# RegulatoryGenomicsGroup/chicdiff

Hardware: AMD Instinct MI355X
Metric: interactions/sec NB-GLM Wald test (higher is better)
Workload: dtype f64; 1 GPU; synthetic 2000000 interactions x 8 samples (4v4), size factors + offsets(theta=0.5) + dispersions + Wald, design ~condition; rows_per_gpu=2000000, samples=8, global_rows=2000000, parallelism=rows-sharded x1, collectives=none (single rank), ranks_in_communicator=1

## Files before the change

chicdiff_amd/csrc/api.hip:

```cpp
#include <math.h>
#include <stdarg.h>
#include <stdio.h>
#include <stdlib.h>
#include <string.h>

#include <algorithm>
#include <mutex>
#include <thread>
#include <string>
#include <vector>
#include <unordered_set>

#include <dlfcn.h>

#include "common.h"
#include "philox.h"
#include "prior_mc.h"

using namespace cd;

namespace cd {
struct ChinputCols {
    std::vector<int32_t> bait, oe, N;
    std::string error;
};
int64_t chinput_parse(const char *path, int nthreads, ChinputCols &c);
}

struct KTimer {
    std::string name;
    hipEvent_t e0 = nullptr, e1 = nullptr;
    double ms = 0;
    int launches = 0;
    double bytes = 0;
};

struct HostOpts {
    int select_all_rounds = 0;
    int trend_one_launch_per_pass = 0;
    int sharded_trend_gather = 1;
    int trend_mad_in_kernel = 1;
    int local_trend_substitute = 1;
    int fuse_offsets = 1;
    int prep_blocks = 0;
    int theta_grid_concurrency = 5;
    int host_copy_threads = 12;
    int bench_fake_world = 0;
    int fault_inject = 0;
    int region_assemble_generic = 0;
    int chicago_tables_run_merge = 1;
};

struct chicdiff_hip_ctx {
    int device = 0;
    bool no_persistent_trend = false;
    Opts tune{};
    HostOpts host;
    char *tg_buf = nullptr;
    size_t tg_bytes = 0;
    double shard_n[kSelMaxWorld] = {0};
    bool shard_n_valid = false;
    int64_t tg_total = 0;
    double *tg_x = nullptr, *tg_y = nullptr, *tg_resid = nullptr;
    int32_t *tg_flags = nullptr;
    int32_t *h_flag = nullptr;
    FusedOffsets fuse;
    int refits = 0;
    bool sf_overflow_seen = false;
    int32_t *d_carry = nullptr;
    char *io_dev = nullptr, *io_pin = nullptr;
    size_t io_dev_bytes = 0, io_pin_bytes = 0;
    ChinputCols *chin = nullptr;
    struct EarlyCopy {
        int n = 0;
        struct Item { int col; char *pin; size_t bytes; } item[10];
        hipEvent_t ready = nullptr, done = nullptr;
        bool issued = false;
    } *early = nullptr;
    hipStream_t copy_stream = nullptr;
    hipEvent_t ev_fork = nullptr, ev_join = nullptr;
    std::vector<chicdiff_hip_ctx *> lanes;
    int cu_count = 0;
    hipStream_t own_stream = nullptr, stream = nullptr;
    chicdiff_allreduce_fn allreduce = nullptr;
    void *allreduce_user = nullptr;
    chicdiff_allgather_fn allgather = nullptr;
    void *allgather_user = nullptr;
    int world = 1, rank = 0;
    void *rccl_lib = nullptr, *rccl_comm = nullptr;
    int (*rccl_allreduce)(const void *, void *, size_t, int, int, void *, hipStream_t) = nullptr;
    int (*rccl_allgather)(const void *, void *, size_t, int, void *, hipStream_t) = nullptr;
    int (*rccl_comm_destroy)(void *) = nullptr;
    const char *(*rccl_error_string)(int) = nullptr;
    char err[512] = {0};
    int64_t cap_n = 0;
    int cap_S = 0;
    void *ws = nullptr;
// ... 39 lines not shown
    va_end(ap);
    return code;
}
#define HIPCHK(c, call)                                                                              \
    do {                                                                                             \
        hipError_t e_ = (call);                                                                      \
        if (e_ != hipSuccess) return fail(c, CHICDIFF_E_HIP, "%s: %s", #call, hipGetErrorString(e_)); \
    } while (0)

extern "C" {

const char *chicdiff_hip_last_error(const chicdiff_hip_ctx *ctx) { return ctx ? ctx->err : g_create_err; }

void chicdiff_hip_default_opts(chicdiff_nbglm_opts *o) {
    o->minDisp = 1e-8;
    o->dispTol = 1e-6;
    o->kappa0 = 1.0;
    o->maxit = 100;
    o->betaMaxit = 100;
    o->betaTol = 1e-8;
    o->minmu = 0.5;
    o->outlierSD = 2.0;
    o->dispPriorVar = NAN;
    o->trendCoef[0] = o->trendCoef[1] = NAN;
    o->fitType = 0;
    o->_pad = 0;
}

struct OptionDef {
    const char *name;
    int32_t Opts::*tune;
    int HostOpts::*host;
    int64_t lo, hi, no_lo, no_hi;
};
static const OptionDef kOptions[] = {
    {"line_search_spread", &Opts::spread, nullptr, 0, 3, 1, 0},
    {"line_search_min_waves", &Opts::min_waves, nullptr, 0, 4, 1, 1},
    {"line_search_chunk", &Opts::chunk, nullptr, 0, 64, 1, 7},
    {"line_search_prio", &Opts::prio, nullptr, 0, 100, 1, 0},
    {"line_search_schedule", &Opts::schedule, nullptr, 0, 4, 2, 2},
    {"line_search_deal", &Opts::deal, nullptr, 0, 64, 1, 0},
    {"line_search_classes_a", &Opts::classes_a, nullptr, 0, 6, 1, 0},
    {"line_search_fillers", &Opts::fillers, nullptr, -1, 1, 1, 0},
    {"line_search_filler_stop", &Opts::filler_stop, nullptr, -1, 100, 1, 0},
    {"theta_grid_concurrency", nullptr, &HostOpts::theta_grid_concurrency, 1, 16, 1, 0},
    {"host_copy_threads", nullptr, &HostOpts::host_copy_threads, 1, 64, 1, 0},
    {"select_all_rounds", nullptr, &HostOpts::select_all_rounds, 0, 1, 1, 0},
    {"trend_one_launch_per_pass", nullptr, &HostOpts::trend_one_launch_per_pass, 0, 1, 1, 0},
    {"sharded_trend_gather", nullptr, &HostOpts::sharded_trend_gather, 0, 1, 1, 0},
    {"trend_persistent_blocks", &Opts::trend_blocks, nullptr, 0, 256, 1, 0},
    {"trend_mad_in_kernel", nullptr, &HostOpts::trend_mad_in_kernel, 0, 1, 1, 0},
    {"fuse_offsets", nullptr, &HostOpts::fuse_offsets, 0, 2, 1, 0},
    {"prep_blocks", nullptr, &HostOpts::prep_blocks, 0, kRedBlocks, 1, 0},
    {"region_assemble_generic", nullptr, &HostOpts::region_assemble_generic, 0, 1, 1, 0},
    {"chicago_tables_run_merge", nullptr, &HostOpts::chicago_tables_run_merge, 0, 1, 1, 0},
    {"fault_inject", nullptr, &HostOpts::fault_inject, 0, 7, 1, 0},
    {"bench_fake_world", nullptr, &HostOpts::bench_fake_world, 0, kGatherMaxWorld, 1, 0},
    {"local_trend_substitute", nullptr, &HostOpts::local_trend_substitute, 0, 1, 1, 0},
};

int chicdiff_hip_set_option(chicdiff_hip_ctx *c, const char *name, int64_t value) {
    if (!c || !name) return CHICDIFF_E_INVALID;
    for (const OptionDef &d : kOptions) {
        if (strcmp(name, d.name) != 0 || value < d.lo || value > d.hi || (value >= d.no_lo && value <= d.no_hi)) continue;
        if (d.host == &HostOpts::bench_fake_world && value > 1 && !getenv("CHICDIFF_BENCH_FAKE_WORLD"))
            return fail(c, CHICDIFF_E_INVALID, "set_option: bench_fake_world is a rehearsal hook of bench.py (CHICDIFF_BENCH_FAKE_WORLD unset)");
        if (d.tune) c->tune.*d.tune = (int32_t)value;
        else c->host.*d.host = (int)value;
        return CHICDIFF_OK;
    }
    return fail(c, CHICDIFF_E_INVALID, "set_option: unknown option or value (%s = %lld)", name, (long long)value);
}

int chicdiff_hip_create(chicdiff_hip_ctx **out, int32_t device) {
    if (!out) return fail(nullptr, CHICDIFF_E_INVALID, "ctx out pointer is NULL");
    *out = nullptr;
    int ndev = 0;
    hipError_t e = hipGetDeviceCount(&ndev);
    if (e != hipSuccess || ndev <= 0)
        return fail(nullptr, CHICDIFF_E_HIP, "no HIP device available (%s): the HIP path cannot run, and there is no CPU fallback",
                    e != hipSuccess ? hipGetErrorString(e) : "device count 0");
    if (device < 0 || device >= ndev) return fail(nullptr, CHICDIFF_E_INVALID, "device %d out of range [0,%d)", device, ndev);
    chicdiff_hip_ctx *c = new chicdiff_hip_ctx();
    c->device = device;
    if ((e = hipSetDevice(device)) != hipSuccess || (e = hipStreamCreateWithFlags(&c->own_stream, hipStreamNonBlocking)) != hipSuccess ||
        (e = hipHostMalloc((void **)&c->h_sc, sizeof(FitScalars))) != hipSuccess ||
        (e = hipHostMalloc((void **)&c->h_sf, sizeof(double) * (kMaxS + 1))) != hipSuccess ||
        (e = hipMalloc((void **)&c->d_sf, sizeof(double) * (kMaxS + 1 + kSelMaxWorld + 8))) != hipSuccess ||
        (e = hipMemset(c->d_sf, 0, sizeof(double) * (kMaxS + 1 + kSelMaxWorld + 8))) != hipSuccess ||
        (e = hipMalloc((void **)&c->d_logfact, sizeof(double) * kLogFactN)) != hipSuccess) {
        fail(nullptr, CHICDIFF_E_HIP, "context setup: %s", hipGetErrorString(e));
        delete c;
        return CHICDIFF_E_HIP;
    }
    {
        hipDeviceProp_t prop;
        if (hipGetDeviceProperties(&prop, device) == hipSuccess) c->cu_count = prop.multiProcessorCount;
    }
    {
        std::vector<double> lf(kLogFactN);
        for (int k = 0; k < kLogFactN; k++) lf[k] = lgamma((double)k + 1.0);
        if ((e = hipMemcpy(c->d_logfact, lf.data(), sizeof(double) * kLogFactN, hipMemcpyHostToDevice)) != hipSuccess) {
            fail(nullptr, CHICDIFF_E_HIP, "context setup: %s", hipGetErrorString(e));
            chicdiff_hip_destroy(c);
            return CHICDIFF_E_HIP;
        }
// ... 786 lines not shown
    }
    if (c->host.fault_inject & 2) {
        c->host.fault_inject &= ~2;
        launch_poke(&w.sc->failed, 3, st);
    }
    const bool mad_local = c->allreduce && c->tg_total > 0;
    FitDims dm = d;
    FitWork wm = w;
    if (mad_local) {
        dm.n = c->tg_total;
        wm.baseMean = c->tg_x;
        wm.dispGene = c->tg_y;
        wm.allZero = c->tg_flags;
        wm.resid = c->tg_resid;
    }
    if (mad_in_kernel) {
        if (prior_by_simulation(d, o) && (rc = prior_mc(c, d, dm, wm, mad_local))) return rc;
    } else {
        launch_dispfit_resid(dm, wm, o, st);
        SelArgs sa{};
        sa.n = dm.n;
        sa.ncol = 1;
        sa.resid = wm.resid;
        Scope t(c, "mad_select");
        sa.mode = SEL_RESID;
        if ((rc = run_select(c, sa, all_rounds, mad_local))) return rc;
        sa.mode = SEL_ABSDEV;
        if ((rc = run_select(c, sa, all_rounds, mad_local))) return rc;
        if (!prior_by_simulation(d, o)) launch_prior_var(d, w, o, st);
        else if ((rc = prior_mc(c, d, dm, wm, mad_local))) return rc;
    }
    if (c->host.fault_inject & 1) {
        c->host.fault_inject &= ~1;
        launch_poke(&w.sc->sel_overflow, 1, st);
    }
    {
        Scope t(c, "disp_map");
        launch_disp_map(d_counts, d_nf, d, w, o, st);
    }
    if (c->early && c->early->n > 0) {
        const void *src[10] = {w.baseMean, w.baseVar, w.dispGene, w.dispFit, w.dispMAP, w.disp, w.geneIter, w.mapIter, w.outlier, w.allZero};
        HIPCHK(c, hipEventRecord(c->early->ready, st));
        HIPCHK(c, hipStreamWaitEvent(c->copy_stream, c->early->ready, 0));
        for (int k = 0; k < c->early->n; k++)
            HIPCHK(c, hipMemcpyAsync(c->early->item[k].pin, src[c->early->item[k].col], c->early->item[k].bytes, hipMemcpyDeviceToHost, c->copy_stream));
        HIPCHK(c, hipEventRecord(c->early->done, c->copy_stream));
        c->early->issued = true;
    }
    static const chicdiff_nbglm_out none{};
    const chicdiff_nbglm_out &out = d_out ? *d_out : none;
    if (d.p == 2) {
        {
            Scope t(c, "wald_prep");
            launch_wald_prep(d_counts, d_nf, d, w, o, st);
        }
        {
            Scope t(c, "wald_irls");
            launch_wald_irls(d_counts, d_nf, d, w, o, st);
        }
        Scope t(c, "wald_final");
        launch_wald_final(d_counts, d_nf, d, w, o, out, st);
    } else {
        Scope t(c, "wald_intercept");
        launch_wald_intercept(d_counts, d_nf, d, w, o, out, st);
    }
    launch_dev_sum_finish(d, w, c->d_carry, c->d_sf, st);
    if ((rc = do_allreduce(c, w.sc->final_sums, 7))) return rc;
    if ((rc = read_scalars(c))) return rc;
    HIPCHK(c, hipGetLastError());
    return CHICDIFF_OK;
}

static int fit_dev_impl(chicdiff_hip_ctx *c, const int32_t *d_counts, const double *d_nf, FitDims d, Opts o,
                        const chicdiff_nbglm_out *d_out, chicdiff_nbglm_scalars *scalars, bool all_rounds) {
    WorkRedirect redirect(c, d_out);
    const double *hs = c->h_sc->final_sums;
    for (;;) {
        if (int rc = fit_pass(c, d_counts, d_nf, d, o, d_out, all_rounds)) return rc;
        if (hs[4] > 0)
            return fail(c, CHICDIFF_E_INVALID, c->h_sc->neg_counts ? "counts contain a negative value or NA_integer_"
                                                                   : "counts contain a negative value or NA_integer_ (on another rank of the sharded fit)");
        c->sf_overflow_seen = hs[6] > 0;
        if (c->sf_overflow_seen && !all_rounds) return CHICDIFF_OK;
        if (hs[5] > 0 && !all_rounds) {
            all_rounds = true;
        } else if (c->h_sc->failed == 3 || hs[3] > 0) {
            if (c->no_persistent_trend) return fail(c, CHICDIFF_E_HIP, "trend fit: grid barrier timed out");
            c->no_persistent_trend = true;
        } else if (c->h_sc->failed && o.fit_type == 0 && !(o.trendIn[0] == o.trendIn[0]) && c->host.local_trend_substitute) {
            o.fit_type = 2;
        } else
            break;
        c->refits++;
    }
    if (scalars) {
        const FitScalars *s = c->h_sc;
        int status = 0;
        if (s->failed) status |= CHICDIFF_ST_TREND_FAILED;
        if (s->trend_local) status |= CHICDIFF_ST_TREND_LOCAL;
        scalars->trendCoef[0] = s->coefs[0];
        scalars->trendCoef[1] = s->coefs[1];
        scalars->varLogDispEsts = s->varLogDispEsts;
        scalars->dispPriorVar = s->dispPriorVar;
        scalars->nAllZero = (int64_t)hs[2];
        scalars->sumDeviance = hs[2] > 0 ? NAN : hs[0];
        scalars->trendOuterIter = s->outer_it;
        if (hs[2] > 0) status |= CHICDIFF_ST_ALLZERO_ROWS;
        if (hs[1] > 0) status |= CHICDIFF_ST_BETA_NONCONV;
        if (prior_by_simulation(d, o)) status |= CHICDIFF_ST_PRIORVAR_MC;
        scalars->status = status;
    }
    return CHICDIFF_OK;
}

static int begin_call(chicdiff_hip_ctx *c, int rc, int64_t n, int32_t S) {
    timing_reset(c);
    if ((rc = shard_consensus(c, rc, n))) return rc;
// ... 1091 lines not shown
```

chicdiff_amd/csrc/common.h:

```cpp
#pragma once
#include <hip/hip_runtime.h>
#include <stdint.h>

#include "../../include/chicdiff_hip.h"
#include "fit_driver.h"
#include "fit_state.h"

namespace cd {

constexpr int kRedBlocks = 1024;

struct FitDims {
    int64_t n;
    int32_t S, p, nA, nB;
    uint64_t gmask;
};

struct FitWork {
    double *baseMean, *baseVar, *gm0, *gm1, *rough, *binit0, *binit1, *crow;
    double *dispGene, *dispFit, *dispMAP, *disp, *beta0, *beta1, *resid;
    int32_t *allZero, *geneIter, *mapIter, *outlier, *betaIter, *optimConv;
    int32_t *order;
    uint8_t *cls;
    int32_t *gridlist;
// ... 94 lines not shown
    __shared__ unsigned int s_cnt[NC];
    if (threadIdx.x < NC) s_cnt[threadIdx.x] = 0;
    __syncthreads();
#pragma unroll
    for (int k = 0; k < NC; k++) {
        unsigned int v = mine[k];
        for (int off = 32; off > 0; off >>= 1) v += __shfl_down(v, off);
        if ((threadIdx.x & 63) == 0 && v) atomicAdd(&s_cnt[k], v);
    }
    __syncthreads();
    if (threadIdx.x < NC) hist[threadIdx.x * kSchedBlocks + blockIdx.x] = s_cnt[threadIdx.x];
}
__device__ __forceinline__ void class_peers(int c, bool valid, int lane, unsigned int &rank, unsigned int &count) {
    unsigned long long m = __ballot(valid);
#pragma unroll
    for (int b = 0; b < 5; b++) {
        const bool bit = (c >> b) & 1;
        const unsigned long long set = __ballot(bit);
        m &= bit ? set : ~set;
    }
    rank = __popcll(m & ((1ull << lane) - 1ull));
    count = __popcll(m);
}
#endif

struct FusedOffsets { const double *fm = nullptr; const double *sf = nullptr; double theta = 0; int mix = 0; };
int launch_prep(const int32_t *counts, double *nf, FitDims d, FitWork w, Opts o, hipStream_t st, FusedOffsets fo = FusedOffsets(), int max_blocks = 0);
void launch_prep_finish(FitDims d, FitWork w, int nblk, double *slot, hipStream_t st);
void launch_xim(FitDims d, FitWork w, const double *slots, int world, hipStream_t st);
void launch_disp_gene(const int32_t *counts, const double *nf, FitDims d, FitWork w, Opts o, hipStream_t st);
void launch_order_build(FitDims d, FitWork w, int classesA, bool have_hist, hipStream_t st, bool fine = false);
void launch_disp_map(const int32_t *counts, const double *nf, FitDims d, FitWork w, Opts o, hipStream_t st);
void launch_trend_persistent(FitDims d, FitWork w, Opts o, hipStream_t st, bool with_mad);
int trend_persistent_blocks();
void launch_trend_init(FitDims d, FitWork w, Opts o, hipStream_t st);
int trend_blocks();
void launch_trend_pass(FitDims d, FitWork w, Opts o, hipStream_t st, bool fused_step);
void launch_trend_step(FitDims d, FitWork w, Opts o, hipStream_t st);
constexpr int kLfMaxV = 100;
struct LfVerts { int nv; int _pad; double x[kLfMaxV], f[kLfMaxV], d[kLfMaxV]; };
void launch_lf_hist(FitDims d, FitWork w, Opts o, int use_dist, double xv, uint64_t prefix, int shift, double *hist, hipStream_t st);
void launch_lf_sums(FitDims d, FitWork w, Opts o, double xv, double h, double *partials, double *out8, hipStream_t st);
void launch_lf_eval(FitDims d, FitWork w, const LfVerts &v, hipStream_t st);
void launch_trend_gather(FitDims d, FitWork w, Opts o, double *xg, double *yg, hipStream_t st);
constexpr int kGatherMaxWorld = 64;
struct GatherLayout { int32_t world, _pad; int64_t block, maxn; int64_t off[kGatherMaxWorld + 1]; };
void launch_trend_compact(const GatherLayout &gl, const double *recv, double *xg, double *yg, hipStream_t st);
void launch_poke(int32_t *p, int32_t v, hipStream_t st);
void launch_flag_to_double(const int32_t *flag, double *out, hipStream_t st);
void launch_dispfit_resid(FitDims d, FitWork w, Opts o, hipStream_t st);
void launch_prior_var(FitDims d, FitWork w, Opts o, hipStream_t st);
void launch_resid_hist(FitDims d, FitWork w, double *out40, hipStream_t st);
void launch_prior_mc(FitDims d, FitWork w, const double *hist40, const void *table, hipStream_t st);
void launch_wald_prep(const int32_t *counts, const double *nf, FitDims d, FitWork w, Opts o, hipStream_t st);
void launch_wald_irls(const int32_t *counts, const double *nf, FitDims d, FitWork w, Opts o, hipStream_t st);
void launch_wald_final(const int32_t *counts, const double *nf, FitDims d, FitWork w, Opts o,
                       const chicdiff_nbglm_out &out, hipStream_t st);
void launch_wald_intercept(const int32_t *counts, const double *nf, FitDims d, FitWork w, Opts o,
                           const chicdiff_nbglm_out &out, hipStream_t st);
void launch_dev_sum_finish(FitDims d, FitWork w, const int32_t *carry, const double *sf_dev, hipStream_t st);

struct SelArgs {
    int mode;
    int ncol;
    int64_t n;
    const double *resid;
    const double *ratio;
    int S;
    int shift;
    double *sf_out;
    int32_t *overflow_out;
};
void launch_sel_hist(SelArgs a, FitWork w, hipStream_t st);
void launch_sel_step(SelArgs a, FitWork w, hipStream_t st);
void launch_sel_shortcut(SelArgs a, FitWork w, hipStream_t st);
void launch_sel_finish(SelArgs a, FitWork w, hipStream_t st);
void launch_sel_keep_local(SelArgs a, FitWork w, hipStream_t st);
void launch_sel_gather_counts(SelArgs a, FitWork w, int world, int rank, hipStream_t st);
void launch_sel_gather_place(SelArgs a, FitWork w, int world, int rank, hipStream_t st);
void launch_sel_gather_finish(SelArgs a, FitWork w, int world, int rank, hipStream_t st);

void launch_row_ratio(const int32_t *counts, int64_t n, int S, double *ratio, int32_t *clear_flag, hipStream_t st);

constexpr double kSfBinLo = -4.0, kSfBinSpan = 8.0;
constexpr int kSfHistWords = 15360;
constexpr int kSfSubBins = 4096;
constexpr int kSfMaxS = 16;
constexpr int kSfWorkWords = kSfHistWords + 2 * kSfMaxS * 32;
__host__ __device__ inline int sf_bins(int S) { return kSfHistWords / (S <= 4 ? 4 : S <= 8 ? 8 : 16); }
__host__ __device__ inline double sf_bin_pos(double x, int nb) { return (x - kSfBinLo) * ((double)nb / kSfBinSpan); }
__host__ __device__ inline int sf_bin(double x, int nb) {
    const double u = floor(sf_bin_pos(x, nb));
    return u < 0.0 ? 0 : (u > (double)(nb - 1) ? nb - 1 : (int)u);
}
__host__ __device__ inline int sf_sub_bin(double x, int nb, int b) {
    const double u = floor((sf_bin_pos(x, nb) - (double)b) * (double)kSfSubBins);
    return u < 0.0 ? 0 : (u > (double)(kSfSubBins - 1) ? kSfSubBins - 1 : (int)u);
}
void launch_sf_direct(const int32_t *counts, int64_t n, int S, SelArgs a, FitWork w, unsigned int *hist, uint64_t *lists,
                      int32_t *clear_flag, int cus, hipStream_t st);
void launch_offsets(const double *fullMean, const double *sf_dev, int64_t n, int S, double theta, int mix,
                    double *out, hipStream_t st);
void launch_window_sums(const int32_t *fragN, const double *fragFM, int64_t nfrag, int S, const int64_t *rptr,
                        int64_t n, int32_t *N, double *FM, hipStream_t st);
size_t count_join_scratch_bytes(int64_t nkeys);
void launch_count_join(const int32_t *bait, const int32_t *oe, int64_t nru, const int64_t *keys,
                       const int32_t *vals, int64_t nkeys, int32_t *out, void *scratch, hipStream_t st);
void launch_fragment_background(const int32_t *bait, const int32_t *oe, int64_t nru, int32_t id_min, int32_t nid,
                                const int64_t *midsum, int32_t S, const double *sj, const double *si, const int32_t *tblb,
                                const int32_t *tlb, const double *T, int32_t ntblb, int32_t ntlb, const double *distfun_dev,
                                double *bmean, double *tmean, double *fullmean, hipStream_t st);
size_t bh_workspace_bytes(int64_t n);
// ... 100 lines not shown
```

chicdiff_amd/csrc/wald_kernels.hip:

```cpp
#include "common.h"
#include "devmath.h"

namespace cd {

constexpr double kLog2e = 1.4426950408889634074;

__global__ __launch_bounds__(256) void wald_prep_kernel(const int32_t *__restrict__ counts,
                                                        const double *__restrict__ nf, FitDims d, FitWork w, int sched, int64_t tile, unsigned int *hist) {
    __shared__ double s_logfact[kLogFactN];
    __shared__ LogEntry s_lt[64];
    for (int k = threadIdx.x; k < kLogFactN; k += 256) s_logfact[k] = w.logfact[k];
    log_table_to_lds(s_lt);
    const int64_t n = d.n;
    const int S = d.S;
    unsigned int mine[kSchedClasses] = {0, 0, 0, 0, 0, 0};
    const int64_t lo = tile > 0 ? (int64_t)blockIdx.x * tile : (int64_t)blockIdx.x * 256;
    const int64_t hi = tile > 0 ? (lo + tile < n ? lo + tile : n) : n;
    const int64_t step = tile > 0 ? 256 : (int64_t)gridDim.x * 256;
    for (int64_t i = lo + threadIdx.x; i < hi; i += step) {
        if (w.allZero[i]) {
            reinterpret_cast<double2 *>(w.start)[2 * i] = make_double2(NAN, 0.0);
            if (sched) {
                w.cls[i] = 255;
                w.beta0[i] = NAN;
// ... 373 lines not shown
            }
            WDIAG(const unsigned long long wt2 = __builtin_amdgcn_s_memtime(); if (sec_bulk) { cyw[sec + 0] += wt1 - wt0; cyw[sec + 1] += wt2 - wt1; cyw[sec + 3]++; wt_eval_end = wt2; })
            const double zA = fma(etaA - 1.0, wA, uA) + zcA, zB = fma(etaB - 1.0, wB, uB) + zcB;
            const double D = (Dl - fma(etaA, syA, etaB * syB)) + Dc;
            bool stop = false;
            int iter_out = k;
            if (k >= 1) {
                const double dev = 2.0 * (D - crow);
                const double diff = fabs(dev - dev_old), scale = fabs(dev) + 0.1;
                if (!(diff == diff) || !(scale == scale) || (isinf(diff) && isinf(scale))) {
                    stop = true;
                    iter_out = o.betaMaxit;
                } else if (k >= 2 && diff < o.betaTol * scale) {
                    stop = true;
                } else if (k >= o.betaMaxit) {
                    stop = true;
                }
                dev_old = dev;
            }
            if (!stop) {
                const double m00 = wA + wB + lambda, m01 = wB, m11 = wB + lambda;
                const double r0 = zA + zB, r1 = zB;
                const double idet = rcp(fma(m00, m11, -(m01 * m01)));
                b0 = fma(m11, r0, -(m01 * r1)) * idet;
                b1 = fma(m00, r1, -(m01 * r0)) * idet;
                k++;
                if (fabs(b0) > 30.0 || fabs(b1) > 30.0) {
                    stop = true;
                    iter_out = o.betaMaxit;
                }
            }
            if (stop) {
                if (iter_out >= o.betaMaxit) {
                    b0 = A.w.binit0[row];
                    b1 = A.w.binit1[row];
                    A.w.optimConv[row] = optim_row(s_y + lane, s_nf + lane, 64, S, gmask, alpha, A.w.crow[row], b0, b1) ? 1 : 0;
                }
                A.w.beta0[row] = b0;
                A.w.beta1[row] = b1;
                A.w.betaIter[row] = iter_out;
                need = true;
            }
        }
        WDIAG(if (wt_eval_end) { cyw[sec + 2] += __builtin_amdgcn_s_memtime() - wt_eval_end; wt_eval_end = 0; })
    }
    WDIAG(if (lane == 0) { for (int q = 0; q < 8; q++) atomicAdd(&g_irls_cy[q], cyw[q]); atomicAdd(&g_irls_open[0], g_open_cy); atomicAdd(&g_irls_open[1], g_open_n); })
}


__device__ __forceinline__ int trim_lo(int n) {
    const double tr = n <= 3 ? 1.0 / 3 : (n <= 23 ? 1.0 / 4 : 1.0 / 8);
    return (int)floor(n * tr);
}
__device__ __forceinline__ double trim_scale(int n) { return n <= 3 ? 2.04 : (n <= 23 ? 1.86 : 1.51); }

__device__ __forceinline__ double cell_trimmed_mean(const double *s_q, int T, int tid, int S, uint64_t gmask, int c,
                                                    int nc, int lo, bool sq, double cm) {
    double sum = 0;
    if (lo == 1) {
        int imin = -1, imax = -1;
        double vmin = INFINITY, vmax = -INFINITY;
        for (int j = 0; j < S; j++) {
            if ((int)((gmask >> j) & 1) != c) continue;
            double vj = s_q[j * T + tid];
            if (sq) vj = (vj - cm) * (vj - cm);
            if (vj < vmin) { vmin = vj; imin = j; }
            if (vj >= vmax) { vmax = vj; imax = j; }
        }
        for (int j = 0; j < S; j++) {
            if ((int)((gmask >> j) & 1) != c || j == imin || j == imax) continue;
            double vj = s_q[j * T + tid];
            if (sq) vj = (vj - cm) * (vj - cm);
            sum += vj;
        }
        return sum / (nc - 2);
    }
    for (int j = 0; j < S; j++) {
        if ((int)((gmask >> j) & 1) != c) continue;
        double vj = s_q[j * T + tid];
        if (sq) vj = (vj - cm) * (vj - cm);
        int rank = 0;
        for (int k = 0; k < S; k++) {
            if ((int)((gmask >> k) & 1) != c) continue;
            double vk = s_q[k * T + tid];
            if (sq) vk = (vk - cm) * (vk - cm);
            rank += (vk < vj || (vk == vj && k < j)) ? 1 : 0;
        }
        if (rank >= lo && rank < nc - lo) sum += vj;
    }
    return sum / (nc - 2 * lo);
}

__global__ __launch_bounds__(256) void wald_final_kernel(const int32_t *__restrict__ counts,
                                                         const double *__restrict__ nf, FitDims d, FitWork w, Opts o,
                                                         chicdiff_nbglm_out out) {
    extern __shared__ double s_q[];
    __shared__ LogEntry s_lt[64];
    __shared__ ExpEntry s_et[64];
    exp_table_to_lds(s_et);
    log_table_to_lds(s_lt);
    const int T = blockDim.x, tid = threadIdx.x;
    const int64_t n = d.n;
    const int S = d.S;
    const double lambda = 1e-6 / (0.69314718055994530942 * 0.69314718055994530942);
    const bool want_cooks = out.maxCooks && (d.nA >= 3 || d.nB >= 3);
    double v[3] = {0, 0, 0};
// ... 175 lines not shown
        } else {
            v[2] += 1;
        }
        if (out.log2FoldChange) out.log2FoldChange[i] = NAN;
        if (out.lfcSE) out.lfcSE[i] = NAN;
        if (out.stat) out.stat[i] = st;
        if (out.pvalue) out.pvalue[i] = pv;
        if (out.intercept) out.intercept[i] = B0;
        if (out.interceptSE) out.interceptSE[i] = s0;
        if (out.deviance) out.deviance[i] = dv;
        if (out.maxCooks) out.maxCooks[i] = NAN;
        if (out.betaConv) out.betaConv[i] = az ? 0 : 1;
        if (out.betaIter) out.betaIter[i] = az ? 0 : 1;
        if (out.cooksArgmax) out.cooksArgmax[i] = -1;
    }
    __shared__ double red[3][4];
    const int lane = threadIdx.x & 63, wave = threadIdx.x >> 6;
    for (int k = 0; k < 3; k++) {
        double x = v[k];
        for (int off = 32; off > 0; off >>= 1) x += __shfl_down(x, off);
        if (lane == 0) red[k][wave] = x;
    }
    __syncthreads();
    if (threadIdx.x < 3)
        w.partials[(size_t)blockIdx.x * 3 + threadIdx.x] =
            (red[threadIdx.x][0] + red[threadIdx.x][1]) + (red[threadIdx.x][2] + red[threadIdx.x][3]);
}

__global__ void dev_sum_kernel(FitWork w, const int32_t *carry, const double *sf_dev, int S) {
    __shared__ double red[256];
    double *sums = w.sc->final_sums;
    for (int k = 0; k < 3; k++) {
        double acc = 0;
        for (int b = threadIdx.x; b < kRedBlocks; b += 256) acc += w.partials[(size_t)b * 3 + k];
        red[threadIdx.x] = acc;
        __syncthreads();
        for (int s = 128; s > 0; s >>= 1) {
            if ((int)threadIdx.x < s) red[threadIdx.x] += red[threadIdx.x + s];
            __syncthreads();
        }
        if (threadIdx.x == 0) sums[k] = red[0];
        __syncthreads();
    }
    if (threadIdx.x == 0) {
        sums[3] = w.sc->failed == 3 ? 1.0 : 0.0;
        sums[4] = w.sc->neg_counts ? 1.0 : 0.0;
        sums[5] = w.sc->sel_overflow ? 1.0 : 0.0;
        sums[6] = (carry && *carry) ? 1.0 : 0.0;
        sums[7] = 0.0;
    }
    if (sf_dev && (int)threadIdx.x < S) w.sc->final_sf[threadIdx.x] = sf_dev[threadIdx.x];
}

static bool irls_schedule(const FitDims &d, const Opts &o) { return o.schedule && d.n > 131072; }
void launch_wald_prep(const int32_t *counts, const double *nf, FitDims d, FitWork w, Opts o, hipStream_t st) {
    o.schedule = irls_schedule(d, o) ? o.schedule : 0;
    int64_t nblk, tile;
    order_tiles(d.n, nblk, tile);
    if (o.schedule && tile == 256) {
        wald_prep_kernel<<<(unsigned)nblk, 256, 0, st>>>(counts, nf, d, w, o.schedule, tile, reinterpret_cast<unsigned int *>(w.hist));
        launch_order_build(d, w, 0, true, st);
        return;
    }
    wald_prep_kernel<<<1536, 256, 0, st>>>(counts, nf, d, w, o.schedule, 0, nullptr);
    if (o.schedule) launch_order_build(d, w, 0, false, st);
}
void launch_wald_irls(const int32_t *counts, const double *nf, FitDims d, FitWork w, Opts o, hipStream_t st) {
    WaldArgs A{counts, nf, d, w, o, 64, irls_schedule(d, o) ? w.order : nullptr, o.spread};
    const size_t lds_per_wave = (size_t)d.S * 64 * 12;
    int threads = 256;
    while (threads > 64 && lds_per_wave * (threads / 64) > 40 * 1024) threads >>= 1;
    const size_t lds = lds_per_wave * (threads / 64);
    int64_t blocks = ((d.n + 63) / 64 + threads / 64 - 1) / (threads / 64);
    int64_t per_cu = (int64_t)(160 * 1024 / lds) < 8 ? (int64_t)(160 * 1024 / lds) : 8;
    const int64_t by_regs = 4 * WALD_MINW / (threads / 64);
    if (per_cu > by_regs) per_cu = by_regs;
    if (blocks > 256 * per_cu) blocks = 256 * per_cu;
    if (blocks < 1) blocks = 1;
    const int64_t per_wave = d.n / (blocks * (threads / 64));
    A.chunk = per_wave >= 256 ? 128 : 64;
#ifdef CHICDIFF_DIAG
    const bool stamps = getenv("CHICDIFF_IRLS_STAMPS") != nullptr;
    if (stamps) {
        unsigned long long z[8] = {0, 0, 0, 0, 0, 0, 0, 0};
        (void)hipMemcpyToSymbol(HIP_SYMBOL(g_irls_cy), z, sizeof z);
        (void)hipMemcpyToSymbol(HIP_SYMBOL(g_irls_open), z, 16);
    }
#endif
    wald_irls_kernel<<<(unsigned)blocks, threads, lds, st>>>(A);
#ifdef CHICDIFF_DIAG
    if (stamps) {
        (void)hipStreamSynchronize(st);
        unsigned long long h[8];
        (void)hipMemcpyFromSymbol(h, HIP_SYMBOL(g_irls_cy), sizeof h);
        {
            const double t = h[3] ? (double)h[3] : 1.0, r = h[7] ? (double)h[7] : 1.0;
            printf("  IRLS ticks while the queue has rows (lane 0 of every wave): %.0f per wave; s_memtime cycles per tick: refill %.0f, evaluate %.0f, solve + state %.0f\n",
                   t / (double)(blocks * (threads / 64)), h[0] / t, h[1] / t, h[2] / t);
            unsigned long long ho[2];
            (void)hipMemcpyFromSymbol(ho, HIP_SYMBOL(g_irls_open), sizeof ho);
            printf("    pieces of the schedule opened: %.1f per wave, %.0f cycles each\n", (double)ho[1] / (double)(blocks * (threads / 64)), ho[1] ? (double)ho[0] / (double)ho[1] : 0.0);
            printf("    inside a refill that lane 0 took part in (%.0f per wave): tick start -> loads issued %.0f, loads issued -> row in LDS %.0f, -> end of the attempt %.0f cycles\n",
                   r / (double)(blocks * (threads / 64)), h[4] / r, h[5] / r, h[6] / r);
        }
    }
#endif
}
void launch_wald_final(const int32_t *counts, const double *nf, FitDims d, FitWork w, Opts o,
                       const chicdiff_nbglm_out &out, hipStream_t st) {
    const int threads = d.S <= 16 ? 256 : 64;
    wald_final_kernel<<<kRedBlocks, threads, (size_t)d.S * threads * sizeof(double), st>>>(counts, nf, d, w, o, out);
}
void launch_wald_intercept(const int32_t *counts, const double *nf, FitDims d, FitWork w, Opts,
                           const chicdiff_nbglm_out &out, hipStream_t st) {
    wald_intercept_kernel<<<kRedBlocks, 256, 0, st>>>(counts, nf, d, w, out);
}
void launch_dev_sum_finish(FitDims d, FitWork w, const int32_t *carry, const double *sf_dev, hipStream_t st) {
    dev_sum_kernel<<<1, 256, 0, st>>>(w, carry, sf_dev, d.S);
}

}
```

Baseline: 590.7 million interactions/s.

## Add sample-count-templated Wald prep, final and intercept kernels with occupancy-sized grids

Adds specialised Wald prep, final and intercept kernels templated on a padded sample count (4/8/16). Per-row counts and size factors are loaded into registers with unrolled loops, and the Cook's trimmed mean uses a branchless min/max drop when only one element is trimmed. Grids are sized from occupancy queries instead of fixed block counts. The aim is to cut generic per-sample loops, LDS traffic and register pressure in the Wald stages, at the cost of more code paths and new options (on by default).

```diff
diff --git a/chicdiff_amd/csrc/api.hip b/chicdiff_amd/csrc/api.hip
--- a/chicdiff_amd/csrc/api.hip
+++ b/chicdiff_amd/csrc/api.hip
@@ -43,6 +43,8 @@
     int local_trend_substitute = 1;
     int fuse_offsets = 1;
     int prep_blocks = 0;
+    int wald_classes = 1;
+    int wald_blocks = 0;
     int theta_grid_concurrency = 5;
     int host_copy_threads = 12;
     int bench_fake_world = 0;
@@ -188,6 +190,8 @@
     {"trend_mad_in_kernel", nullptr, &HostOpts::trend_mad_in_kernel, 0, 1, 1, 0},
     {"fuse_offsets", nullptr, &HostOpts::fuse_offsets, 0, 2, 1, 0},
     {"prep_blocks", nullptr, &HostOpts::prep_blocks, 0, kRedBlocks, 1, 0},
+    {"wald_classes", nullptr, &HostOpts::wald_classes, 0, 1, 1, 0},
+    {"wald_blocks", nullptr, &HostOpts::wald_blocks, 0, kRedBlocks, 1, 0},
     {"region_assemble_generic", nullptr, &HostOpts::region_assemble_generic, 0, 1, 1, 0},
     {"chicago_tables_run_merge", nullptr, &HostOpts::chicago_tables_run_merge, 0, 1, 1, 0},
     {"fault_inject", nullptr, &HostOpts::fault_inject, 0, 7, 1, 0},
@@ -1080,17 +1084,17 @@
     if (d.p == 2) {
         {
             Scope t(c, "wald_prep");
-            launch_wald_prep(d_counts, d_nf, d, w, o, st);
+            launch_wald_prep(d_counts, d_nf, d, w, o, st, c->host.wald_classes, c->host.wald_blocks);
         }
         {
             Scope t(c, "wald_irls");
             launch_wald_irls(d_counts, d_nf, d, w, o, st);
         }
         Scope t(c, "wald_final");
-        launch_wald_final(d_counts, d_nf, d, w, o, out, st);
+        launch_wald_final(d_counts, d_nf, d, w, o, out, st, c->host.wald_classes, c->host.wald_blocks);
     } else {
         Scope t(c, "wald_intercept");
-        launch_wald_intercept(d_counts, d_nf, d, w, o, out, st);
+        launch_wald_intercept(d_counts, d_nf, d, w, o, out, st, c->host.wald_classes);
     }
     launch_dev_sum_finish(d, w, c->d_carry, c->d_sf, st);
     if ((rc = do_allreduce(c, w.sc->final_sums, 7))) return rc;
diff --git a/chicdiff_amd/csrc/common.h b/chicdiff_amd/csrc/common.h
--- a/chicdiff_amd/csrc/common.h
+++ b/chicdiff_amd/csrc/common.h
@@ -170,12 +170,12 @@
 void launch_prior_var(FitDims d, FitWork w, Opts o, hipStream_t st);
 void launch_resid_hist(FitDims d, FitWork w, double *out40, hipStream_t st);
 void launch_prior_mc(FitDims d, FitWork w, const double *hist40, const void *table, hipStream_t st);
-void launch_wald_prep(const int32_t *counts, const double *nf, FitDims d, FitWork w, Opts o, hipStream_t st);
+void launch_wald_prep(const int32_t *counts, const double *nf, FitDims d, FitWork w, Opts o, hipStream_t st, int classes = 1, int max_blocks = 0);
 void launch_wald_irls(const int32_t *counts, const double *nf, FitDims d, FitWork w, Opts o, hipStream_t st);
 void launch_wald_final(const int32_t *counts, const double *nf, FitDims d, FitWork w, Opts o,
-                       const chicdiff_nbglm_out &out, hipStream_t st);
+                       const chicdiff_nbglm_out &out, hipStream_t st, int classes = 1, int max_blocks = 0);
 void launch_wald_intercept(const int32_t *counts, const double *nf, FitDims d, FitWork w, Opts o,
-                           const chicdiff_nbglm_out &out, hipStream_t st);
+                           const chicdiff_nbglm_out &out, hipStream_t st, int classes = 1);
 void launch_dev_sum_finish(FitDims d, FitWork w, const int32_t *carry, const double *sf_dev, hipStream_t st);
 
 struct SelArgs {
diff --git a/chicdiff_amd/csrc/wald_kernels.hip b/chicdiff_amd/csrc/wald_kernels.hip
--- a/chicdiff_amd/csrc/wald_kernels.hip
+++ b/chicdiff_amd/csrc/wald_kernels.hip
@@ -449,6 +449,7 @@
     const double tr = n <= 3 ? 1.0 / 3 : (n <= 23 ? 1.0 / 4 : 1.0 / 8);
     return (int)floor(n * tr);
 }
+static int trim_lo_host(int n) { return n <= 3 ? 1 : (n <= 23 ? n / 4 : n / 8); }
 __device__ __forceinline__ double trim_scale(int n) { return n <= 3 ? 2.04 : (n <= 23 ? 1.86 : 1.51); }
 
 __device__ __forceinline__ double cell_trimmed_mean(const double *s_q, int T, int tid, int S, uint64_t gmask, int c,
@@ -730,9 +731,418 @@
     if (sf_dev && (int)threadIdx.x < S) w.sc->final_sf[threadIdx.x] = sf_dev[threadIdx.x];
 }
 
+template <int N> constexpr int kWaldPrepWaves = N == 16 ? 2 : 3;
+template <int N> constexpr int kWaldFinalWaves = N == 16 ? 2 : 4;
+template <int N> constexpr int kWaldInterceptWaves = N == 4 ? 3 : 2;
+template <int N, typename V>
+__device__ __forceinline__ void wald_load(const V *__restrict__ src, int64_t n, int S, int64_t i, V (&v)[N]) {
+#pragma unroll
+    for (int j = 0; j < N; j++) v[j] = src[(int64_t)(j < S ? j : S - 1) * n + i];
+}
+
+__device__ __forceinline__ void wald_design(const FitDims &d, int &S, uint32_t &gbits) {
+    S = d.S;
+    gbits = (uint32_t)d.gmask;
+    asm volatile("" : "+s"(S), "+s"(gbits));
+}
+
+template <int N>
+__device__ __forceinline__ void wald_prep_row(const int32_t *__restrict__ counts, const double *__restrict__ nf, const FitDims &d, const FitWork &w,
+                                              int sched, int64_t i, const double *s_logfact, const LogEntry *s_lt, unsigned int (&mine)[kSchedClasses]) {
+    const int64_t n = d.n;
+    int S;
+    uint32_t gbits;
+    wald_design(d, S, gbits);
+    int32_t yv[N];
+    double fv[N];
+    wald_load<N>(counts, n, S, i, yv);
+    wald_load<N>(nf, n, S, i, fv);
+    if (w.allZero[i]) {
+        reinterpret_cast<double2 *>(w.start)[2 * i] = make_double2(NAN, 0.0);
+        if (sched) {
+            w.cls[i] = 255;
+            w.beta0[i] = NAN;
+            w.beta1[i] = NAN;
+            w.betaIter[i] = 0;
+        }
+        return;
+    }
+    const double alpha = w.disp[i], la = flog(alpha);
+    if (sched) {
+        const double gmin = fmin(w.gm0[i], w.gm1[i]);
+        const int cl = gmin < 0.5 ? 0 : (gmin < 1.0 ? 1 : ((gmin < 2.0 || alpha > 1.5) ? 2 : 3));
+        w.cls[i] = (uint8_t)cl;
+#pragma unroll
+        for (int k = 0; k < kSchedClasses; k++) mine[k] += (cl == k);
+    }
+    const LgrCtx cs = lgr_make_t(rcp(alpha), s_lt), c1 = lgr_one();
+    double lA = 0, lB = 0, c = 0, cst = 0;
+#pragma unroll
+    for (int j = 0; j < N; j++) {
+        if (j < S) {
+            const int yi = yv[j];
+            const double nfj = fv[j];
+            const double l = tlog((double)yi / nfj + 0.1, s_lt);
+            if ((gbits >> j) & 1u) lB += l; else lA += l;
+            if (yi > 0) {
+                c += lgr_eval_t(cs, yi, s_lt) - (yi < kLogFactN ? s_logfact[yi] : lgr_eval(c1, yi));
+                cst = fma((double)yi, la + tlog(nfj, s_lt), cst);
+            }
+            __builtin_amdgcn_sched_barrier(0);
+        }
+    }
+    lA /= d.nA;
+    lB /= d.nB;
+    w.binit0[i] = lA;
+    w.binit1[i] = lB - lA;
+    w.crow[i] = c;
+    double2 *h = reinterpret_cast<double2 *>(w.start) + 2 * i;
+    h[0] = make_double2(alpha, c + cst);
+    h[1] = make_double2(lA, lB - lA);
+}
+
+template <int N>
+__global__ __launch_bounds__(256, kWaldPrepWaves<N>) void wald_prep_class_kernel(const int32_t *__restrict__ counts, const double *__restrict__ nf, FitDims d, FitWork w,
+                                                              int sched, int64_t tile, int ntiles, unsigned int *hist) {
+    __shared__ double s_logfact[kLogFactN];
+    __shared__ LogEntry s_lt[64];
+    __shared__ unsigned int s_cnt[kSchedClasses];
+    for (int k = threadIdx.x; k < kLogFactN; k += 256) s_logfact[k] = w.logfact[k];
+    log_table_to_lds(s_lt);
+    const int64_t n = d.n;
+    unsigned int mine[kSchedClasses] = {0, 0, 0, 0, 0, 0};
+    if (tile == 0) {
+        for (int64_t i = (int64_t)blockIdx.x * 256 + threadIdx.x; i < n; i += (int64_t)gridDim.x * 256)
+            wald_prep_row<N>(counts, nf, d, w, sched, i, s_logfact, s_lt, mine);
+        return;
+    }
+    for (int tb = blockIdx.x; tb < ntiles; tb += gridDim.x) {
+        const int64_t lo = (int64_t)tb * tile, hi = lo + tile < n ? lo + tile : n;
+#pragma unroll
+        for (int k = 0; k < kSchedClasses; k++) mine[k] = 0;
+        for (int64_t i = lo + threadIdx.x; i < hi; i += 256) wald_prep_row<N>(counts, nf, d, w, sched, i, s_logfact, s_lt, mine);
+        if (threadIdx.x < kSchedClasses) s_cnt[threadIdx.x] = 0;
+        __syncthreads();
+#pragma unroll
+        for (int k = 0; k < kSchedClasses; k++) {
+            unsigned int v = mine[k];
+            for (int off = 32; off > 0; off >>= 1) v += __shfl_down(v, off);
+            if ((threadIdx.x & 63) == 0 && v) atomicAdd(&s_cnt[k], v);
+        }
+        __syncthreads();
+        if (threadIdx.x < kSchedClasses) hist[threadIdx.x * kSchedBlocks + tb] = s_cnt[threadIdx.x];
+    }
+}
+
+template <int N, bool SQ, bool LDS>
+__device__ __forceinline__ double class_trimmed_mean1(const double *q, int S, uint32_t gbits, int c, int nc, double cm) {
+    double t[N];
+    int imin = -1, imax = -1;
+    double vmin = INFINITY, vmax = -INFINITY;
+#pragma unroll
+    for (int j = 0; j < N; j++) t[j] = q[LDS ? (j < S ? j : S - 1) * 256 : j];
+#pragma unroll
+    for (int j = 0; j < N; j++) {
+        const bool in = j < S && (int)((gbits >> j) & 1u) == c;
+        double vj = t[j];
+        if (SQ) vj = (vj - cm) * (vj - cm);
+        t[j] = vj;
+        const bool lt = in && vj < vmin, ge = in && vj >= vmax;
+        vmin = lt ? vj : vmin;
+        imin = lt ? j : imin;
+        vmax = ge ? vj : vmax;
+        imax = ge ? j : imax;
+    }
+    double sum = 0;
+#pragma unroll
+    for (int j = 0; j < N; j++) {
+        const bool in = j < S && (int)((gbits >> j) & 1u) == c;
+        sum = (in && j != imin && j != imax) ? sum + t[j] : sum;
+    }
+    return sum / (nc - 2);
+}
+
+template <int N, bool RANK>
+__global__ __launch_bounds__(256, kWaldFinalWaves<N>) void wald_final_class_kernel(const int32_t *__restrict__ counts, const double *__restrict__ nf, FitDims d, FitWork w,
+                                                               Opts o, chicdiff_nbglm_out out) {
+    constexpr bool LEAN = N == 8, QLDS = LEAN || RANK;
+    extern __shared__ double s_q[];
+    __shared__ LogEntry s_lt[64];
+    __shared__ ExpEntry s_et[64];
+    __shared__ double red[3][4];
+    exp_table_to_lds(s_et);
+    log_table_to_lds(s_lt);
+    const int tid = threadIdx.x, lane = threadIdx.x & 63, wave = threadIdx.x >> 6;
+    const int64_t n = d.n;
+    const double lambda = 1e-6 / (0.69314718055994530942 * 0.69314718055994530942);
+    const bool want_cooks = out.maxCooks && (d.nA >= 3 || d.nB >= 3);
+    for (int vb = blockIdx.x; vb < kRedBlocks; vb += gridDim.x) {
+        if ((int64_t)vb * 256 >= n) {
+            if (tid < 3) w.partials[(size_t)vb * 3 + tid] = 0.0;
+            continue;
+        }
+        double vdev = 0;
+        int nbad = 0, nzero = 0;
+        for (int64_t i = (int64_t)vb * 256 + tid; i < n; i += (int64_t)kRedBlocks * 256) {
+            int S;
+            uint32_t gbits;
+            wald_design(d, S, gbits);
+            int32_t yv[N];
+            double fv[N];
+            wald_load<N>(counts, n, S, i, yv);
+            wald_load<N>(nf, n, S, i, fv);
+            const bool az = w.allZero[i];
+            double B0 = NAN, B1 = NAN, s0 = NAN, s1 = NAN, st = NAN, pv = NAN, dv = NAN, mc = NAN;
+            int bconv = 0, biter = 0, amax = -1;
+            if (!az) {
+                const double alpha = w.disp[i], size = rcp(alpha);
+                const double b0 = w.beta0[i], b1 = w.beta1[i];
+                biter = w.betaIter[i];
+                const int oc = biter < o.betaMaxit ? -1 : w.optimConv[i];
+                bconv = (biter < o.betaMaxit) || oc == 1;
+                const double E0 = texp(b0, s_et), E1 = texp(b0 + b1, s_et);
+                const double la = tlog(alpha, s_lt);
+                double wA = 0, wB = 0, ll = w.crow[i], m = 0;
+                double muv[LEAN ? 1 : N], wv[LEAN ? 1 : N], q[LEAN ? 1 : N];
+                double *s_mu = s_q + S * 256 + tid;
+#pragma unroll
+                for (int j = 0; j < N; j++) {
+                    if (!LEAN) {
+                        muv[j] = 0;
+                        wv[j] = 0;
+                        q[j] = 0;
+                    }
+                    if (j < S) {
+                        const bool g = (gbits >> j) & 1u;
+                        const double y = (double)yv[j];
+                        const double nfj = fv[j];
+                        const double muf = nfj * (g ? E1 : E0);
+                        const double mu = fmax(muf, o.minmu);
+                        const double wj = mu * rcp(fma(alpha, mu, 1.0));
+                        if (g) wB += wj; else wA += wj;
+                        const double mul = oc >= 0 ? mu : muf;
+                        const double ma = alpha * mul, t = 1.0 + ma;
+                        ll -= (size + y) * tlog1p_from(ma, t, rcp(t), s_lt);
+                        if (y > 0) ll += y * (la + tlog(mul, s_lt));
+                        if (!LEAN) {
+                            muv[j] = muf;
+                            wv[j] = wj;
+                        }
+                        if (want_cooks) {
+                            if (LEAN) s_mu[j * 256] = muf;
+                            const double qj = y / nfj;
+                            if (!LEAN) q[j] = qj;
+                            if (QLDS) s_q[j * 256 + tid] = qj;
+                            m += qj;
+                        }
+                        __builtin_amdgcn_sched_barrier(0);
+                    }
+                }
+                const double m00 = wA + wB + lambda, m01 = wB, m11 = wB + lambda, det = m00 * m11 - m01 * m01;
+                const double idet = rcp_or_div(det);
+                const double i00 = m11 * idet, i01 = -m01 * idet, i11 = m00 * idet;
+                const double a00 = wA + wB, a01 = wB, a11 = wB;
+                const double t00 = i00 * a00 + i01 * a01, t01 = i00 * a01 + i01 * a11;
+                const double t10 = i01 * a00 + i11 * a01, t11 = i01 * a01 + i11 * a11;
+                const double v0 = t00 * i00 + t01 * i01, v1 = t10 * i01 + t11 * i11;
+                B0 = kLog2e * b0;
+                B1 = kLog2e * b1;
+                s0 = kLog2e * sqrt(fmax(v0, 0.0));
+                s1 = kLog2e * sqrt(fmax(v1, 0.0));
+                st = B1 / s1;
+                pv = pnorm_two_sided(st);
+                dv = -2.0 * ll;
+                if (!bconv || !(v0 > 0) || !(v1 > 0)) nbad++;
+                __builtin_amdgcn_sched_barrier(0);
+                if (want_cooks) {
+                    m /= S;
+                    double vmax = -INFINITY;
+#pragma unroll
+                    for (int c = 0; c < 2; c++) {
+                        const int nc = c ? d.nB : d.nA;
+                        if (nc < 3) continue;
+                        const int lo = trim_lo(nc);
+                        double cm, cv;
+                        if (!RANK || lo == 1) {
+                            cm = class_trimmed_mean1<N, false, LEAN>(LEAN ? s_q + tid : q, S, gbits, c, nc, 0.0);
+                            cv = class_trimmed_mean1<N, true, LEAN>(LEAN ? s_q + tid : q, S, gbits, c, nc, cm);
+                        } else {
+                            cm = cell_trimmed_mean(s_q, 256, tid, S, d.gmask, c, nc, lo, false, 0.0);
+                            cv = cell_trimmed_mean(s_q, 256, tid, S, d.gmask, c, nc, lo, true, cm);
+                        }
+                        const double vv = trim_scale(nc) * cv;
+                        if (vv > vmax) vmax = vv;
+                        __builtin_amdgcn_sched_barrier(0);
+                    }
+                    const double arob = fmax((vmax - m) / (m * m), 0.04);
+                    mc = -INFINITY;
+                    double call = -INFINITY;
+#pragma unroll
+                    for (int j = 0; j < N; j++) {
+                        if (j < S) {
+                            const bool g = (gbits >> j) & 1u;
+                            const double yc = (double)yv[j];
+                            const double muf = LEAN ? s_mu[j * 256] : muv[j];
+                            const double wj = LEAN ? fmax(muf, o.minmu) * rcp(fma(alpha, fmax(muf, o.minmu), 1.0)) : wv[j];
+                            const double h = wj * (g ? (i00 + 2 * i01 + i11) : i00);
+                            const double V = muf + arob * muf * muf;
+                            const double ck = ((yc - muf) * (yc - muf) * 0.5 * h) * rcp_or_div(V * ((1 - h) * (1 - h)));
+                            if (ck > call) { call = ck; amax = j; }
+                            if ((g ? d.nB : d.nA) >= 3 && ck > mc) mc = ck;
+                            __builtin_amdgcn_sched_barrier(0);
+                        }
+                    }
+                }
+                vdev += dv;
+            } else {
+                nzero++;
+            }
+            if (out.log2FoldChange) out.log2FoldChange[i] = B1;
+            if (out.lfcSE) out.lfcSE[i] = s1;
+            if (out.stat) out.stat[i] = st;
+            if (out.pvalue) out.pvalue[i] = pv;
+            if (out.intercept) out.intercept[i] = B0;
+            if (out.interceptSE) out.interceptSE[i] = s0;
+            if (out.deviance) out.deviance[i] = dv;
+            if (out.maxCooks) out.maxCooks[i] = mc;
+            if (out.betaConv) out.betaConv[i] = bconv;
+            if (out.betaIter) out.betaIter[i] = biter;
+            if (out.cooksArgmax) out.cooksArgmax[i] = amax;
+        }
+        __syncthreads();
+        const double v[3] = {vdev, (double)nbad, (double)nzero};
+        for (int k = 0; k < 3; k++) {
+            double x = v[k];
+            for (int off = 32; off > 0; off >>= 1) x += __shfl_down(x, off);
+            if (lane == 0) red[k][wave] = x;
+        }
+        __syncthreads();
+        if (tid < 3) {
+            double acc = 0;
+            for (int q4 = 0; q4 < 4; q4++) acc += red[tid][q4];
+            w.partials[(size_t)vb * 3 + tid] = acc;
+        }
+    }
+}
+
+template <int N>
+__global__ __launch_bounds__(256, kWaldInterceptWaves<N>) void wald_intercept_class_kernel(const int32_t *__restrict__ counts, const double *__restrict__ nf, FitDims d,
+                                                                   FitWork w, chicdiff_nbglm_out out) {
+    __shared__ double s_logfact[kLogFactN];
+    __shared__ LogEntry s_lt[64];
+    for (int k = threadIdx.x; k < kLogFactN; k += 256) s_logfact[k] = w.logfact[k];
+    log_table_to_lds(s_lt);
+    const int64_t n = d.n;
+    double v[3] = {0, 0, 0};
+    for (int64_t i = blockIdx.x * 256 + threadIdx.x; i < n; i += (int64_t)gridDim.x * 256) {
+        int S;
+        uint32_t gbits;
+        wald_design(d, S, gbits);
+        int32_t yv[N];
+        double f[N];
+        wald_load<N>(counts, n, S, i, yv);
+        wald_load<N>(nf, n, S, i, f);
+        double B0 = NAN, s0 = NAN, st = NAN, pv = NAN, dv = NAN;
+        const bool az = w.allZero[i];
+        if (!az) {
+            const double alpha = w.disp[i], size = rcp(alpha);
+            double bm = 0;
+#pragma unroll
+            for (int j = 0; j < N; j++)
+                if (j < S) bm += (double)yv[j] / f[j];
+            bm /= S;
+            B0 = log2(bm);
+            const double e = exp2(B0);
+            const LgrCtx cs = lgr_make_t(size, s_lt), c1 = lgr_one();
+            const double la = tlog(alpha, s_lt);
+            double ll = 0, xtwx = 0;
+#pragma unroll
+            for (int j = 0; j < N; j++)
+                if (j < S) {
+                    const double nfj = f[j];
+                    const int yi = yv[j];
+                    const double mu = nfj * e;
+                    const double y = (double)yi, ma = alpha * mu, t = 1.0 + ma, rt = rcp(t);
+                    ll -= (size + y) * tlog1p_from(ma, t, rt, s_lt);
+                    if (yi > 0) ll += lgr_eval_t(cs, yi, s_lt) - (yi < kLogFactN ? s_logfact[yi] : lgr_eval(c1, yi)) + y * (la + tlog(mu, s_lt));
+                    xtwx += mu * rt;
+                    __builtin_amdgcn_sched_barrier(0);
+                }
+            s0 = kLog2e * sqrt(1.0 / xtwx);
+            st = B0 / s0;
+            pv = pnorm_two_sided(st);
+            dv = -2.0 * ll;
+            v[0] += dv;
+        } else {
+            v[2] += 1;
+        }
+        if (out.log2FoldChange) out.log2FoldChange[i] = NAN;
+        if (out.lfcSE) out.lfcSE[i] = NAN;
+        if (out.stat) out.stat[i] = st;
+        if (out.pvalue) out.pvalue[i] = pv;
+        if (out.intercept) out.intercept[i] = B0;
+        if (out.interceptSE) out.interceptSE[i] = s0;
+        if (out.deviance) out.deviance[i] = dv;
+        if (out.maxCooks) out.maxCooks[i] = NAN;
+        if (out.betaConv) out.betaConv[i] = az ? 0 : 1;
+        if (out.betaIter) out.betaIter[i] = az ? 0 : 1;
+        if (out.cooksArgmax) out.cooksArgmax[i] = -1;
+    }
+    __shared__ double red[3][4];
+    const int lane = threadIdx.x & 63, wave = threadIdx.x >> 6;
+    for (int k = 0; k < 3; k++) {
+        double x = v[k];
+        for (int off = 32; off > 0; off >>= 1) x += __shfl_down(x, off);
+        if (lane == 0) red[k][wave] = x;
+    }
+    __syncthreads();
+    if (threadIdx.x < 3)
+        w.partials[(size_t)blockIdx.x * 3 + threadIdx.x] =
+            (red[threadIdx.x][0] + red[threadIdx.x][1]) + (red[threadIdx.x][2] + red[threadIdx.x][3]);
+}
+
+template <typename K>
+static int wald_resident(K kernel, size_t lds) {
+    int per_cu = 0, dev = 0, cus = 0;
+    if (hipOccupancyMaxActiveBlocksPerMultiprocessor(&per_cu, kernel, 256, lds) != hipSuccess || per_cu < 1) per_cu = 4;
+    if (per_cu > 8) per_cu = 8;
+    if (hipGetDevice(&dev) != hipSuccess || hipDeviceGetAttribute(&cus, hipDeviceAttributeMultiprocessorCount, dev) != hipSuccess || cus < 1) cus = 256;
+    (void)hipGetLastError();
+    return per_cu * cus;
+}
+template <int N>
+static void wald_prep_class_launch(const int32_t *counts, const double *nf, FitDims d, FitWork w, int sched, int max_blocks, hipStream_t st) {
+    static const int resident = wald_resident(wald_prep_class_kernel<N>, 0);
+    int64_t ntiles = 0, tile = 0;
+    if (sched) order_tiles(d.n, ntiles, tile);
+    const bool ride = sched && (tile == 256 || ntiles <= resident);
+    int64_t blocks = ride ? ntiles : (d.n + 255) / 256;
+    if (blocks > resident) blocks = resident;
+    if (max_blocks > 0 && blocks > max_blocks) blocks = max_blocks;
+    if (blocks < 1) blocks = 1;
+    wald_prep_class_kernel<N><<<(unsigned)blocks, 256, 0, st>>>(counts, nf, d, w, sched, ride ? tile : 0, (int)ntiles, reinterpret_cast<unsigned int *>(w.hist));
+    if (sched) launch_order_build(d, w, 0, ride, st);
+}
+template <int N, bool RANK>
+static void wald_final_class_launch(const int32_t *counts, const double *nf, FitDims d, FitWork w, Opts o, const chicdiff_nbglm_out &out,
+                                    int max_blocks, hipStream_t st) {
+    constexpr bool QLDS = RANK || N == 8;
+    constexpr size_t cols = N == 8 ? 2 : 1;
+    static const int resident = wald_resident(wald_final_class_kernel<N, RANK>, QLDS ? cols * N * 256 * sizeof(double) : 0);
+    int blocks = resident < kRedBlocks ? resident : kRedBlocks;
+    if (max_blocks > 0 && blocks > max_blocks) blocks = max_blocks;
+    wald_final_class_kernel<N, RANK><<<blocks, 256, QLDS ? cols * d.S * 256 * sizeof(double) : 0, st>>>(counts, nf, d, w, o, out);
+}
+
 static bool irls_schedule(const FitDims &d, const Opts &o) { return o.schedule && d.n > 131072; }
-void launch_wald_prep(const int32_t *counts, const double *nf, FitDims d, FitWork w, Opts o, hipStream_t st) {
+void launch_wald_prep(const int32_t *counts, const double *nf, FitDims d, FitWork w, Opts o, hipStream_t st, int classes, int max_blocks) {
     o.schedule = irls_schedule(d, o) ? o.schedule : 0;
+    if (classes && d.S <= 16) {
+        if (d.S <= 4) wald_prep_class_launch<4>(counts, nf, d, w, o.schedule, max_blocks, st);
+        else if (d.S <= 8) wald_prep_class_launch<8>(counts, nf, d, w, o.schedule, max_blocks, st);
+        else wald_prep_class_launch<16>(counts, nf, d, w, o.schedule, max_blocks, st);
+        return;
+    }
     int64_t nblk, tile;
     order_tiles(d.n, nblk, tile);
     if (o.schedule && tile == 256) {
@@ -785,12 +1195,31 @@
 #endif
 }
 void launch_wald_final(const int32_t *counts, const double *nf, FitDims d, FitWork w, Opts o,
-                       const chicdiff_nbglm_out &out, hipStream_t st) {
+                       const chicdiff_nbglm_out &out, hipStream_t st, int classes, int max_blocks) {
+    if (classes && d.S <= 16) {
+        const bool rank = (d.nA >= 3 && trim_lo_host(d.nA) != 1) || (d.nB >= 3 && trim_lo_host(d.nB) != 1);
+        if (d.S > 8) {
+            if (rank) wald_final_class_launch<16, true>(counts, nf, d, w, o, out, max_blocks, st);
+            else wald_final_class_launch<16, false>(counts, nf, d, w, o, out, max_blocks, st);
+            return;
+        }
+        if (!rank) {
+            if (d.S <= 4) wald_final_class_launch<4, false>(counts, nf, d, w, o, out, max_blocks, st);
+            else wald_final_class_launch<8, false>(counts, nf, d, w, o, out, max_blocks, st);
+            return;
+        }
+    }
     const int threads = d.S <= 16 ? 256 : 64;
     wald_final_kernel<<<kRedBlocks, threads, (size_t)d.S * threads * sizeof(double), st>>>(counts, nf, d, w, o, out);
 }
 void launch_wald_intercept(const int32_t *counts, const double *nf, FitDims d, FitWork w, Opts,
-                           const chicdiff_nbglm_out &out, hipStream_t st) {
+                           const chicdiff_nbglm_out &out, hipStream_t st, int classes) {
+    if (classes && d.S <= 16) {
+        if (d.S <= 4) wald_intercept_class_kernel<4><<<kRedBlocks, 256, 0, st>>>(counts, nf, d, w, out);
+        else if (d.S <= 8) wald_intercept_class_kernel<8><<<kRedBlocks, 256, 0, st>>>(counts, nf, d, w, out);
+        else wald_intercept_class_kernel<16><<<kRedBlocks, 256, 0, st>>>(counts, nf, d, w, out);
+        return;
+    }
     wald_intercept_kernel<<<kRedBlocks, 256, 0, st>>>(counts, nf, d, w, out);
 }
 void launch_dev_sum_finish(FitDims d, FitWork w, const int32_t *carry, const double *sf_dev, hipStream_t st) {
```

Measured after the change: 587.1 million interactions/s. Within noise of the previous version (-0.6%).
